# wvangansbeke/LaneDetection_End2End

Measured on AMD Instinct MI355X. Metric: images/sec fwd+bwd, 256x512 2-lane bs32, higher is better.
Workload: dtype f32; 1 GPU; BEV ERFNet + fused WLS fit + Area loss, 2 lanes, 256x512, batch 32 per GPU, fp32, train mode (BN batch stats, Dropout2d on), fwd+bwd, optimizer excluded; global_batch=32, parallelism=dp1, grad_allreduce=none

## Files before the change

### lanedetection_end2end_amd/_lib.py

```python
import ctypes
import os
from ctypes import c_char_p, c_double, c_int, c_long, c_size_t, c_void_p

import torch

_HERE = os.path.dirname(os.path.abspath(__file__))
LIB_PATH = os.path.join(_HERE, "liblanefit_hip.so")
_lib = None


class LaneFitLibraryError(RuntimeError):
    pass


def _declare(lib):
    P, I, L, D = c_void_p, c_int, c_long, c_double
    sig = {
        "lf_abi_version": (c_int, []),
        "lf_last_error": (c_char_p, []),
        "lf_wls_workspace_bytes": (c_size_t, [I, I, I]),
        "lf_wls_fwd": (I, [P, P, L, I, I, I, I, I, I, D, D, I, I, P, P, P, P, P, P]),
        "lf_wls_bwd": (I, [P, P, L, I, I, I, I, I, I, D, I, P, P, P, P, P]),
        "lf_gels_workspace_bytes": (c_size_t, [I, I]),
        "lf_gels_fwd": (I, [P, P, I, L, I, P, P, P, P, P]),
# ... 86 lines not shown
        "lf_wls_bwd_theta": (I, [P, P, L, P, P, I, I, I, I, I, I, D, I, P, P, P, P, P, P, P]),
        "lf_wls_bwd_grid": (I, [P, P, L, I, I, I, I, I, I, D, I, P, P, P, P, P]),
        "lf_lane_eval": (I, [P, P, P, P, P, P, L, P, I, I, I, I, I, D, D, P, P, P, P, P, P]),
        "lf_lane_decode_bev": (I, [P, I, P, P, P, P, L, P, P, I, D, P, P, I, I, I, I, I, I, I, I, I, I, P, P, P]),
        "lf_step_loss_workspace_bytes": (c_size_t, []),
        "lf_step_loss": (I, [I, I, I, I, I, I, I, P, L, I, P, P, L, I, P, P, P, P, P, P, P, I, D, D, P, P, P, P, P, P]),
        "lf_step_loss_bwd": (I, [P, I, L, L, P, P, P]),
        "lf_seg_step_workspace_bytes": (c_size_t, [I, I, I, I, I, I]),
        "lf_seg_step": (I, [P, P, P, P, L, P, I, I, I, I, I, I, I, D, D, I, P, P, P, P, P, P, P, P]),
        "lf_seg_step_bwd": (I, [P, L, P, P]),
        "lf_label_batch_bp": (I, [P, P, P, P, P, P, P, L, P, P, I, I, P, P, P, P, P, P, P, P, P]),
        "lf_label_batch_bev": (I, [P, P, P, P, P, L, P, P, I, P, P, P, P, P, P, P]),
    }
    dbg = {
        "lf_debug_set_split_any_size": (None, [I]),
        "lf_debug_set_bf16_lds": (None, [I]),
        "lf_debug_set_bf16_no_partial_fast": (None, [I]),
        "lf_debug_stride2_epi": (I, [I, I, P, P, P, P, I, P, P, P, P, I, I, I, I, I, P, P]),
        "lf_debug_set_ops_precision": (None, [I]),
        "lf_debug_conv1d_fwd_phases": (I, [P, P, P, P, I, I, I, I, I, I, P, P, P]),
        "lf_debug_conv1d_wgrad_phases": (I, [P, P, I, I, I, I, I, I, P, P, P]),
        "lf_debug_conv1d_fwd_pro": (I, [P, P, P, P, P, P, I, I, I, I, I, I, P, P]),
        "lf_debug_set_wgrad_ro": (None, [I, I, I]),
        "lf_debug_conv1d_bwd_data_epi3": (I, [P, P, P, P, P, P, P, I, I, I, I, I, I, P, P]),
        "lf_debug_conv1d_epi": (I, [P, P, P, P, I, I, P, P, P, P, P, P, I, I, I, I, I, I, P, P]),
        "lf_debug_conv1d_wgrad_pro": (I, [P, P, P, P, P, P, I, I, I, I, I, I, P, P]),
        "lf_debug_bias_residual_launches": (L, []),
        "lf_debug_partial_fast_launches": (L, []),
    }
    for table in (sig, dbg):
        for name, (res, args) in table.items():
            fn = getattr(lib, name)
            fn.restype = res
            fn.argtypes = args
    return sig


def exported_symbols():
    return list(_declare(load()).keys()) + list(_extra_symbols)


_extra_symbols = []


def load():
    global _lib
# ... 53 lines not shown
```

### lanedetection_end2end_amd/csrc/lf_conv.h

```cpp
#pragma once
#include "lf_common.h"

#define LF_MAX_TAPS 9
struct TapIdx { int v[LF_MAX_TAPS]; };

struct LfTapGeom {
    int N, Hl, Wl;
    int Hs, Ws, s_pix, s_choff;
    int ssh, ssw;
    int Hd, Wd, d_pix, d_choff;
    int dsh, dsw, dah, daw;
    int Cs, Cd;
    int ntaps;
    int tdh[LF_MAX_TAPS], tdw[LF_MAX_TAPS];
};

enum { LF_PRO_NONE = 0, LF_PRO_BNRELU = 1 };
enum {
    LF_EPI_RELU = 1,
    LF_EPI_MASK = 2,
    LF_EPI_ADD = 4,
    LF_EPI_STATS_SQ = 8,
    LF_EPI_MASKBN = 16,
    LF_EPI_STATS_XHAT = 32,
// ... 8 lines not shown
    int split;
    const void* wp48;
    const float* bias;
    float* dst;
    const float* pro_sc;
    const float* pro_sh;
    const float* mask_src;
    const float* add_src;
    const float* aux;
    const float* msc;
    const float* msh;
    const float* asc;
    const float* ash;
    const float* dm;
    float* stats;
    int stats_ld;
    unsigned long long* dbg;
};

void lf_tapgemm_set_split_any_size(int v);
void lf_tapgemm_set_bf16_lds(int v);
void lf_tapgemm_set_bf16_no_partial_fast(int v);
long lf_tapgemm_partial_fast_launches();
int lf_tapgemm_stat_rows(const LfTapGeom& g);
int lf_tapgemm_stat_rows_for(const LfTapGeom& g, const LfTapArgs& a);
int lf_tapgemm_launch(const LfTapGeom& g, const LfTapArgs& a, int pro, int epi, hipStream_t st);
int lf_tapgemm_launch_unordered(const LfTapGeom& g, const LfTapArgs& a, int pro, int epi, hipStream_t st);

struct LfWgradArgs {
    const float* x;
    const float* g;
    const float* pro_sc;
    const float* pro_sh;
    int s16;
    int split;
    float* partial;
    float* bias_partial;
    unsigned long long* dbg = nullptr;
};
int lf_tapwgrad_splits(const LfTapGeom& g);
int lf_tapwgrad_splits_bound(const LfTapGeom& g, int s16);
int lf_tapwgrad_splits_for(const LfTapGeom& g, const LfWgradArgs& a, int pro);
int lf_tapwgrad_launch(const LfTapGeom& g, const LfWgradArgs& a, int pro, hipStream_t st);

bool lf_tapwgrad_ro_ok(const LfTapGeom& g, int s16);
int lf_tapwgrad_ro_rows_bound(const LfTapGeom& g);
// ... 49 lines not shown
```

### lanedetection_end2end_amd/csrc/lf_conv.hip

```cpp
#include <stdlib.h>
#include <string.h>

#include <atomic>
#include <map>
#include <mutex>
#include <tuple>
#include <utility>

#include <hip/hip_ext.h>

#include "lf_conv.h"
#include "lf_ldsdma.h"
#include "lf_types.h"

typedef float f32x4 __attribute__((ext_vector_type(4)));

namespace {

constexpr int MT = 4;
constexpr int WG_WAVES = 4;
constexpr int PIX_PER_WG = WG_WAVES * MT * 16;

__device__ __forceinline__ f32x4 ldg4(const float* p) { return *reinterpret_cast<const f32x4*>(p); }
typedef unsigned u32x4v __attribute__((vector_size(16)));
// ... 51 lines not shown
}
template <int CTRL>
__device__ __forceinline__ float dpp_mov(float v) {
    return __builtin_bit_cast(float, __builtin_amdgcn_update_dpp(0, __builtin_bit_cast(int, v), CTRL, 0xf, 0xf, false));
}
__device__ __forceinline__ f32x4 bcast16(f32x4 v) {
    f32x4 r;
    r.x = dpp_mov<0x150>(v.x); r.y = dpp_mov<0x150>(v.y); r.z = dpp_mov<0x150>(v.z); r.w = dpp_mov<0x150>(v.w);
    return r;
}
__device__ __forceinline__ float sum16(float v) {
    v += dpp_mov<0xB1>(v);
    v += dpp_mov<0x4E>(v);
    v += dpp_mov<0x124>(v);
    v += dpp_mov<0x128>(v);
    return v;
}

#define LF_EPI_GROUPS 1
#define LF_EPI_ONE_TILE false
#define LF_EPI_TID threadIdx.x
#define LF_EPI_ROW1 false
#define LF_EPI_PIVOT true
#define LF_TAPGEMM_EPILOGUE \
      \
    const bool stats = (epi & (LF_EPI_STATS_SQ | LF_EPI_STATS_XHAT)) != 0; \
    constexpr bool NOBIAS = EPIC >= 0 && !(EPIC & LF_EPI_BIAS) && (EPIC & (LF_EPI_MASK | LF_EPI_ADD | LF_EPI_MASKBN | LF_EPI_STATS_XHAT)) != 0; \
    constexpr int NC = (NT % 2 == 0 && !LF_EPI_ONE_TILE) ? 2 : 1; \
     \
    constexpr bool HOISTM = HOISTV && !(EPIC >= 0 && (EPIC & LF_EPI_MASKBN) && (EPIC & LF_EPI_STATS_XHAT)); \
    __builtin_amdgcn_s_setprio(3);    \
    const __amdgpu_buffer_rsrc_t r_dst = make_rsrc(a.dst, 0xffffffffu), r_add = make_rsrc(a.add_src, 0xffffffffu), \
                                 r_msk = make_rsrc(a.mask_src, 0xffffffffu), r_aux = make_rsrc(a.aux, 0xffffffffu), \
                                 r_bias = make_rsrc(a.bias, 0xffffffffu), r_msc = make_rsrc(a.msc, 0xffffffffu), \
                                 r_msh = make_rsrc(a.msh, 0xffffffffu), r_dm = make_rsrc(a.dm, 0xffffffffu); \
     \
    f32x4 s1[NT], s2[NT], bs[NOBIAS ? 1 : NT], hv[HOISTV ? NT : 1][2], piv[LF_EPI_PIVOT ? NT : 1]; \
_Pragma("unroll") \
    for (int n = 0; n < NT; ++n) { \
        const int co = cob + n * 16 + kq * 4; \
        s1[n] = zero4(); s2[n] = zero4(); piv[LF_EPI_PIVOT ? n : 0] = zero4(); \
        if constexpr (!NOBIAS) bs[n] = a.bias ? ldb4(r_bias, co * 4u, 0u) : zero4(); \
        if (HOISTV) { \
            if (HOISTM && (epi & LF_EPI_MASKBN)) { hv[n][0] = ldb4(r_msc, co * 4u, 0u); hv[n][1] = ldb4(r_msh, co * 4u, 0u); } \
        } \
    } \
_Pragma("unroll") \
    for (int m = 0; m < MT; ++m) { \
        const unsigned dbase = (unsigned)(((pn[m] * g.Hd + pi[m] * g.dsh + g.dah) * g.Wd + pj[m] * g.dsw + g.daw) * g.d_pix + g.d_choff + cob + kq * 4); \
_Pragma("unroll") \
        for (int n0 = 0; n0 < NT; n0 += NC) { \
        f32x4 la[NC], lm[NC], lx[NC], ld[NC]; \
_Pragma("unroll") \
        for (int j = 0; j < NC; ++j) { \
            const int n = n0 + j; \
            if (epi & LF_EPI_ADD) la[j] = epi_ld<S16>(r_add, dbase + n * 16); \
            if (epi & LF_EPI_MASK) lm[j] = epi_ld<S16>(r_msk, dbase + n * 16); \
            if (epi & (LF_EPI_MASKBN | LF_EPI_STATS_XHAT)) lx[j] = epi_ld<S16>(r_aux, dbase + n * 16); \
            if ((epi & LF_EPI_STATS_XHAT) && a.dm && !LF_EPI_ROW1) ld[j] = ldb4(r_dm, (unsigned)(pn[m] * g.Cd + cob + n * 16 + kq * 4) * 4u, 0u); \
        } \
_Pragma("unroll") \
        for (int j = 0; j < NC; ++j) { \
            const int n = n0 + j; \
            f32x4 v = acc[n][m]; \
            if constexpr (!NOBIAS) v += bs[n]; \
            if (epi & LF_EPI_ADD) v += la[j]; \
            if (epi & LF_EPI_MASK) v = keep_pos(v, lm[j]); \
            const int co = cob + n * 16 + kq * 4;    \
            if (epi & LF_EPI_MASKBN) v = keep_pos(v, lx[j] * (HOISTM ? hv[HOISTV ? n : 0][0] : ldb4(r_msc, co * 4u, 0u)) + (HOISTM ? hv[HOISTV ? n : 0][1] : ldb4(r_msh, co * 4u, 0u))); \
            if (epi & LF_EPI_RELU) v = S16 ? relu_keep_nan(v) : max0(v); \
            if (S16) v = round_bf16(v);    \
            if (pv[m]) epi_st<S16>(r_dst, dbase + n * 16, v); \
            if (!pv[m]) v = zero4(); \
            if (epi & LF_EPI_STATS_SQ) { \
                if (LF_EPI_PIVOT && m == 0) piv[LF_EPI_PIVOT ? n : 0] = bcast16(v); \
                f32x4 dv = LF_EPI_PIVOT ? v - piv[LF_EPI_PIVOT ? n : 0] : v; \
                if (!pv[m]) dv = zero4(); \
                s1[n] += dv; s2[n] += dv * dv; \
            } \
            if (epi & LF_EPI_STATS_XHAT) { \
                const f32x4 gm = (a.dm && !LF_EPI_ROW1) ? v * ld[j] : v; \
                s1[n] += gm; s2[n] += gm * lx[j];       \
            } \
        } \
        } \
    } \
    if (LF_EPI_ROW1 && (epi & LF_EPI_STATS_XHAT) && a.dm) { \
         \
_Pragma("unroll") \
        for (int n = 0; n < NT; ++n) { \
            const f32x4 dmv = ldb4(r_dm, (unsigned)(pn[0] * g.Cd + cob + n * 16 + kq * 4) * 4u, 0u); \
            s1[n] *= dmv; s2[n] *= dmv; \
        } \
    } \
    if (stats) { \
         \
        const int EW = wave & 3, EG = wave >> 2; \
        __shared__ float sred[LF_EPI_GROUPS][WG_WAVES][NT][4][8]; \
_Pragma("unroll") \
        for (int n = 0; n < NT; ++n) { \
            f32x4 r1, r2; \
            r1.x = sum16(s1[n].x); r1.y = sum16(s1[n].y); r1.z = sum16(s1[n].z); r1.w = sum16(s1[n].w); \
            r2.x = sum16(s2[n].x); r2.y = sum16(s2[n].y); r2.z = sum16(s2[n].z); r2.w = sum16(s2[n].w); \
            if (epi & LF_EPI_STATS_SQ) {       \
                const unsigned lf_t0 = (bx * (unsigned)(WG_WAVES * LF_EPI_GROUPS) + (unsigned)wave) * 64u; \
                const float nw = lf_t0 < npix ? (float)min(npix - lf_t0, 64u) : 0.f; \
                const float rn = nw > 0.f ? 1.f / nw : 0.f; \
                r2 = r2 - r1 * r1 * rn; \
                r2.x = fmaxf(r2.x, 0.f); r2.y = fmaxf(r2.y, 0.f); r2.z = fmaxf(r2.z, 0.f); r2.w = fmaxf(r2.w, 0.f); \
                if (LF_EPI_PIVOT) r1 = r1 + piv[LF_EPI_PIVOT ? n : 0] * nw; \
            } \
            if (pl == 0) { \
                float* d = sred[EG][EW][n][kq]; \
                d[0] = r1.x; d[1] = r1.y; d[2] = r1.z; d[3] = r1.w; d[4] = r2.x; d[5] = r2.y; d[6] = r2.z; d[7] = r2.w; \
            } \
        } \
        __syncthreads(); \
        if ((LF_EPI_TID & 255) < NT * 4 * 8) { \
            const int tg = LF_EPI_TID >> 8, tt = LF_EPI_TID & 255; \
            const int j = tt & 7, q = (tt >> 3) & 3, n = tt >> 5; \
            float v = sred[tg][0][n][q][j] + sred[tg][1][n][q][j] + sred[tg][2][n][q][j] + sred[tg][3][n][q][j]; \
            if ((epi & LF_EPI_STATS_SQ) && j >= 4) {       \
                const unsigned lf_tb = (bx * (unsigned)LF_EPI_GROUPS + (unsigned)tg) * (unsigned)(WG_WAVES * 64); \
                float nwv[4], sw[4], nt = 0.f, st = 0.f; \
_Pragma("unroll") \
                for (int w = 0; w < 4; ++w) { \
                    const unsigned t0w = lf_tb + (unsigned)w * 64u; \
                    nwv[w] = t0w < npix ? (float)min(npix - t0w, 64u) : 0.f; \
                    sw[w] = sred[tg][w][n][q][j - 4]; \
                    nt += nwv[w]; st += sw[w]; \
                } \
                const float mg = nt > 0.f ? st / nt : 0.f; \
_Pragma("unroll") \
                for (int w = 0; w < 4; ++w) \
                    if (nwv[w] > 0.f) { const float dmw = sw[w] / nwv[w] - mg; v += nwv[w] * dmw * dmw; } \
            } \
            const int co = cob + n * 16 + q * 4 + (j & 3); \
            a.stats[((long)(j >> 2) * g.Cd + co) * a.stats_ld + ((long)bx * LF_EPI_GROUPS + tg)] = v;       \
        } \
    } \

extern __shared__ __attribute__((aligned(16))) unsigned char lf_tap_lds[];
constexpr size_t LF_TAP_LDS_PER_TAP = (size_t)WG_WAVES * 64 * (sizeof(uint4) + sizeof(unsigned));

template <int NT, int PROC, int EPIC = -1, bool ROW1 = false, bool DBG = false>
__global__ __launch_bounds__(256, (EPIC >= 0 || NT < 4) ? 2 : 1) void tapgemm_kernel(const LfTapGeom g, const LfTapArgs a, const int pro, const int epi_rt) {
    const int epi = EPIC >= 0 ? EPIC : epi_rt;
    constexpr bool S16 = false, HOISTV = EPIC >= 0;
    unsigned long long tstamp[4] = {0ull, 0ull, 0ull, 0ull};
    if constexpr (DBG) tstamp[0] = __builtin_amdgcn_s_memrealtime();
    const unsigned npix = (unsigned)(g.N * g.Hl * g.Wl);
    const int cob = blockIdx.y * NT * 16;
    const unsigned ntiles = (npix + PIX_PER_WG - 1) / PIX_PER_WG;
    unsigned t_first = blockIdx.x, t_stride = gridDim.x, t_end = ntiles;
    if ((gridDim.x & 7u) == 0 && (ntiles & 7u) == 0) {
        const unsigned per = ntiles >> 3;
        t_first = (blockIdx.x & 7u) * per + (blockIdx.x >> 3); t_stride = gridDim.x >> 3; t_end = (blockIdx.x & 7u) * per + per;
    }
    for (unsigned bx = t_first; bx < t_end; bx += t_stride) {
    unsigned tid = threadIdx.x;
    asm volatile("" : "+v"(tid));
    const int lane = tid & 63, wave = tid >> 6;
    const int pl = lane & 15, kq = lane >> 4;
// ... 171 lines not shown
    LF_TAPGEMM_EPILOGUE
#undef LF_EPI_ONE_TILE
#define LF_EPI_ONE_TILE false
#undef LF_EPI_TID
#define LF_EPI_TID threadIdx.x
#undef LF_EPI_ROW1
#define LF_EPI_ROW1 false
    if (stats && bx + t_stride < t_end) __syncthreads();
    __builtin_amdgcn_s_setprio(0);
    }
    if constexpr (DBG) {
        asm volatile("s_waitcnt vmcnt(0)" ::: "memory");
        tstamp[3] = __builtin_amdgcn_s_memrealtime();
        const int lane = threadIdx.x & 63, wave = threadIdx.x >> 6;
        if (lane == 0 && a.dbg) {
            unsigned long long* d = a.dbg + ((unsigned long long)(blockIdx.y * gridDim.x + blockIdx.x) * WG_WAVES + wave) * 8;
            d[0] = tstamp[0]; d[1] = tstamp[1]; d[2] = tstamp[2]; d[3] = tstamp[3];
            unsigned hwid, xcc;
            asm volatile("s_getreg_b32 %0, hwreg(HW_REG_HW_ID)" : "=s"(hwid));
            asm volatile("s_getreg_b32 %0, hwreg(HW_REG_XCC_ID)" : "=s"(xcc));
            d[4] = (unsigned long long)hwid | ((unsigned long long)xcc << 32);
        }
    }
}

typedef __bf16 bf16x8 __attribute__((ext_vector_type(8)));
typedef unsigned u32x4 __attribute__((ext_vector_type(4)));

__device__ __forceinline__ bf16x8 cvt_bf16x8(f32x4 lo, f32x4 hi) {
    bf16x8 r;
    r[0] = (__bf16)lo.x; r[1] = (__bf16)lo.y; r[2] = (__bf16)lo.z; r[3] = (__bf16)lo.w;
    r[4] = (__bf16)hi.x; r[5] = (__bf16)hi.y; r[6] = (__bf16)hi.z; r[7] = (__bf16)hi.w;
    return r;
}

template <int NT, int PROC, int EPIC = -1, bool FAST = false>
__global__ __launch_bounds__(256, 2) void tapgemm_bf16_kernel(const LfTapGeom g, const LfTapArgs a, const int pro, const int epi_rt) {
    static_assert(!FAST || PROC == 0, "FAST: the out-of-range zero must be the operand itself");
    const int epi = EPIC >= 0 ? EPIC : epi_rt;
    constexpr bool HOISTV = true, S16 = true;
    const int lane = threadIdx.x & 63, wave = threadIdx.x >> 6;
    const int pl = lane & 15, kq = lane >> 4;
    const unsigned npix = (unsigned)(g.N * g.Hl * g.Wl);
    const int cob = blockIdx.y * NT * 16;
    unsigned bx = blockIdx.x;
    if ((gridDim.x & 7u) == 0) bx = (bx & 7u) * (gridDim.x >> 3) + (bx >> 3);
// ... 1356 lines not shown
bool lf_tapgemm_split_ok(const LfTapGeom& g) {
    const long npix = (long)g.N * g.Hl * g.Wl;
    const long wgs = npix / (2 * PIX_PER_WG) * (g.Cd / 64);
    return g.Cs % 32 == 0 && g.Cd % 64 == 0 && g.s_pix % 4 == 0 && g.s_choff % 4 == 0 && npix % (2 * PIX_PER_WG) == 0 &&
           (wgs >= 192 || g_split_any_size);
}

int lf_tapgemm_stat_rows(const LfTapGeom& g) {
    const long npix = (long)g.N * g.Hl * g.Wl;
    return lf_cdiv(npix, PIX_PER_WG);
}
int lf_tapgemm_stat_rows_for(const LfTapGeom& g, const LfTapArgs& a) {
    (void)a;
    return lf_cdiv((long)g.N * g.Hl * g.Wl, PIX_PER_WG);
}

namespace {
std::mutex g_launch_state_mutex;
int current_device() {
    int dev = 0;
    return hipGetDevice(&dev) == hipSuccess ? dev : -1;
}
template <typename K>
int resident_workgroups(K kernel, size_t lds) {
    static std::map<std::tuple<int, const void*, size_t>, int> cache;
    const int dev = current_device();
    const std::tuple<int, const void*, size_t> key(dev, reinterpret_cast<const void*>(kernel), lds);
    std::lock_guard<std::mutex> lock(g_launch_state_mutex);
    auto it = cache.find(key);
    if (it != cache.end()) return it->second;
    int cus = 0, nb = 0;
    if (dev < 0 || hipDeviceGetAttribute(&cus, hipDeviceAttributeMultiprocessorCount, dev) != hipSuccess ||
        hipOccupancyMaxActiveBlocksPerMultiprocessor(&nb, kernel, 256, lds) != hipSuccess || nb < 1 || cus < 1)
        return cache[key] = 1 << 30;
    return cache[key] = nb * cus;
}
bool allow_big_lds(const void* kernel, int bytes) {
    static std::map<std::pair<int, const void*>, bool> done;
    const std::pair<int, const void*> key(current_device(), kernel);
    std::lock_guard<std::mutex> lock(g_launch_state_mutex);
    auto it = done.find(key);
    if (it != done.end()) return it->second;
    return done[key] = hipFuncSetAttribute(kernel, hipFuncAttributeMaxDynamicSharedMemorySize, bytes) == hipSuccess;
}
thread_local unsigned g_launch_flags = 0;
template <typename K>
void launch_tapgemm(K kernel, dim3 grid, size_t lds, hipStream_t st, const LfTapGeom& g, const LfTapArgs& a, int pro, int epi) {
    const unsigned res = (unsigned)resident_workgroups(kernel, lds) / grid.y;
    if (grid.x > res && res >= 8) grid.x = res & ~7u;
    if (g_launch_flags) hipExtLaunchKernelGGL(kernel, grid, dim3(256), (unsigned)lds, st, nullptr, nullptr, g_launch_flags, g, a, pro, epi);
    else hipLaunchKernelGGL(kernel, grid, dim3(256), lds, st, g, a, pro, epi);
}
template <int EPIV, bool DBGV = false>
void launch_bf16_ring(unsigned nitems, hipStream_t st, const LfTapGeom& g, const LfTapArgs& a, int pro, int epi) {
    auto kern = tapgemm_bf16_ring_kernel<EPIV, DBGV>;
    const size_t ring_lds = (size_t)LB_STAGES * LB_STAGE_BYTES;
// ... 4 lines not shown
}
template <int CBV, int EPIV, int PROV = 0>
bool launch_bf16_wl(unsigned nitems, hipStream_t st, const LfTapGeom& g, const LfTapArgs& a, int pro, int epi) {
    auto kern = tapgemm_bf16_wl_kernel<CBV, EPIV, PROV>;
    const size_t lds = WlCfg<CBV, EPIV, PROV>::LDS;
    if (!allow_big_lds(reinterpret_cast<const void*>(kern), 160 * 1024 - 4096)) return false;
    unsigned gx = nitems;
    const unsigned res = (unsigned)resident_workgroups(kern, lds);
    if (gx > res && res >= 8) gx = res & ~7u;
    hipLaunchKernelGGL(kern, dim3(gx), dim3(256), lds, st, g, a, pro, epi);
    return true;
}
template <int EPIV>
bool launch_bf16_wv(unsigned ntiles, hipStream_t st, const LfTapGeom& g, const LfTapArgs& a, int pro, int epi) {
    auto kern = tapgemm_bf16_wv_kernel<EPIV>;
    const size_t lds = WvCfg<EPIV>::LDS;
    if (!allow_big_lds(reinterpret_cast<const void*>(kern), 160 * 1024 - 4096)) return false;
    unsigned gx = ntiles;
    const unsigned res = (unsigned)resident_workgroups(kern, lds);
    if (gx > res && res >= 8) gx = res & ~7u;
    hipLaunchKernelGGL(kern, dim3(gx), dim3(256), lds, st, g, a, pro, epi);
    return true;
}
}

int lf_tapgemm_launch_unordered(const LfTapGeom& g, const LfTapArgs& a, int pro, int epi, hipStream_t st) {
    g_launch_flags = hipExtAnyOrderLaunch;
    const int rc = lf_tapgemm_launch(g, a, pro, epi, st);
    g_launch_flags = 0;
    return rc;
}

int lf_tapgemm_launch(const LfTapGeom& g, const LfTapArgs& a, int pro, int epi, hipStream_t st) {
    LF_REQUIRE(g.Cs % 16 == 0 && g.Cd % 16 == 0, "tapgemm: channels must be multiples of 16 (Cs=%d Cd=%d)", g.Cs, g.Cd);
    LF_REQUIRE(g.s_pix % 4 == 0 && g.s_choff % 4 == 0 && g.d_pix % 4 == 0 && g.d_choff % 4 == 0, "tapgemm: unaligned channel layout");
    LF_REQUIRE(g.ntaps >= 1 && g.ntaps <= LF_MAX_TAPS, "tapgemm: bad tap count %d", g.ntaps);
    const long npix = (long)g.N * g.Hl * g.Wl;
    LF_REQUIRE(npix < (1L << 30), "tapgemm: too many pixels (%ld)", npix);
    const int nt = pick_nt(g.Cd);
    dim3 grid(lf_cdiv(npix, PIX_PER_WG), g.Cd / (16 * nt));
    LF_REQUIRE((long)g.N * g.Hs * g.Ws * g.s_pix * 4 < (long)LF_OOB, "tapgemm: source tensor too large for 32-bit byte offsets");
    LF_REQUIRE((long)g.N * g.Hd * g.Wd * g.d_pix * 4 < (long)LF_OOB, "tapgemm: destination tensor too large for 32-bit byte offsets");
#define LF_TG(NTV)                                                                                                       \
    do {                                                                                                                 \
        if (pro == LF_PRO_BNRELU) launch_tapgemm(tapgemm_kernel<NTV, 1>, grid, tap_lds, st, g, a, pro, epi);  \
        else launch_tapgemm(tapgemm_kernel<NTV, 0>, grid, tap_lds, st, g, a, pro, epi);                       \
    } while (0)
// ... 178 lines not shown
            else if (epis == LF_EPI_STATS_SQ) hipLaunchKernelGGL((tapgemm_bf16_kernel<1, 0, LF_EPI_STATS_SQ, true>), grid, dim3(256), 0, st, g, a, pro, epi);
            else if (epis == LF_EPI_RELU) hipLaunchKernelGGL((tapgemm_bf16_kernel<1, 0, LF_EPI_RELU, true>), grid, dim3(256), 0, st, g, a, pro, epi);
            else hipLaunchKernelGGL((tapgemm_bf16_kernel<1, 0, LF_EPI_ADD, true>), grid, dim3(256), 0, st, g, a, pro, epi);
            if (g.Cs % 32 != 0) ++g_part_fast_launches;
        } else
        switch (nt) {
            case 4: LF_TG16(4); break;
            case 3: LF_TG16(3); break;
            case 2: LF_TG16(2); break;
            default: LF_TG16(1); break;
        }
#undef LF_TG16
#undef LF_TG16F
        LF_CHECK_LAUNCH("tapgemm_bf16");
        return 0;
    }
    if (a.dbg) {
        LF_REQUIRE(nt == 4 && pro == LF_PRO_NONE && epi == 0 && !a.wp16, "tapgemm: phase stamps are compiled into the plain fp32 convolution only");
        if ((g.Wl & 63) == 0) hipLaunchKernelGGL((tapgemm_kernel<4, 0, 0, true, true>), grid, dim3(256), tap_lds, st, g, a, pro, epi);
        else hipLaunchKernelGGL((tapgemm_kernel<4, 0, 0, false, true>), grid, dim3(256), tap_lds, st, g, a, pro, epi);
        LF_CHECK_LAUNCH("tapgemm (stamps)");
        return 0;
    }
    switch (nt) {
        case 4:
            if (pro == LF_PRO_BNRELU && epi == LF_EPI_RELU) LF_TG4(1, LF_EPI_RELU);
            else if (pro == LF_PRO_BNRELU) LF_TG4(1, -1);
            else switch (epis) {
                case 0: LF_TG4(0, 0); break;
                case LF_EPI_RELU: LF_TG4(0, LF_EPI_RELU); break;
                case LF_EPI_MASK: LF_TG4(0, LF_EPI_MASK); break;
                case LF_EPI_ADD: LF_TG4(0, LF_EPI_ADD); break;
                case LF_EPI_STATS_SQ: LF_TG4(0, LF_EPI_STATS_SQ); break;
                case LF_EPI_MASK | LF_EPI_STATS_XHAT: LF_TG4(0, LF_EPI_MASK | LF_EPI_STATS_XHAT); break;
                case LF_EPI_ADD | LF_EPI_MASK | LF_EPI_STATS_XHAT: LF_TG4(0, LF_EPI_ADD | LF_EPI_MASK | LF_EPI_STATS_XHAT); break;
                case LF_EPI_MASKBN | LF_EPI_STATS_XHAT: LF_TG4(0, LF_EPI_MASKBN | LF_EPI_STATS_XHAT); break;
                case BRES: LF_TG4(0, BRES); ++g_bres_launches; break;
                default: LF_TG4(0, -1); break;
            }
            break;
        case 3: LF_TG(3); break;
        case 2: LF_TG(2); break;
        default:
            {
#define LF_LEAN(PROV, EPIV) hipLaunchKernelGGL((tapgemm_lean_kernel<1, PROV, EPIV>), grid, dim3(256), 0, st, g, a, pro, epi)
                if (pro == LF_PRO_BNRELU && epi == LF_EPI_RELU) LF_LEAN(1, LF_EPI_RELU);
// ... 1125 lines not shown
```

### lanedetection_end2end_amd/csrc/lf_debug.h

```cpp
#pragma once
#ifdef __cplusplus
extern "C" {
#endif
void lf_debug_set_split_any_size(int v);
void lf_debug_set_bf16_lds(int v);
void lf_debug_set_bf16_no_partial_fast(int v);
long lf_debug_partial_fast_launches(void);
void lf_debug_set_ops_precision(int mode);
int lf_debug_conv1d_fwd_phases(const float* x, const float* w, const float* bias, float* y, int N, int H, int W, int C,
                               int axis, int dilation, float* scratch, unsigned long long* dbg, void* stream);
int lf_debug_conv1d_fwd_pro(const float* x, const float* w, const float* bias, const float* sc, const float* sh, float* y, int N, int H,
                            int W, int C, int axis, int dilation, float* scratch, void* stream);
void lf_debug_set_wgrad_ro(int mode, int cap64, int cap128);
int lf_debug_conv1d_wgrad_pro(const float* x, const float* gy, const float* sc, const float* sh, float* gw, float* gb, int N, int H, int W,
                              int C, int axis, int dilation, float* scratch, void* stream);
int lf_debug_conv1d_bwd_data_epi3(const float* gy, const float* w, const float* mask_src, const float* add_src, const float* aux,
                                  float* gx, float* stats, int N, int H, int W, int C, int axis, int dilation, float* scratch, void* stream);
int lf_debug_conv1d_epi(const float* src, const float* w, const float* bias, float* dst, int transposed, int epi, const float* mask_src,
                        const float* add_src, const float* aux, const float* msc, const float* msh, float* stats, int N, int H, int W, int C,
                        int axis, int dilation, float* scratch, void* stream);
int lf_debug_stride2_epi(int kind, int phase, const float* src, const float* w, const float* bias, float* dst, int epi, const float* mask_src,
                         const float* add_src, const float* aux, float* stats, int N, int H, int W, int Cin, int Cout, float* scratch,
                         void* stream);
long lf_debug_bias_residual_launches(void);
int lf_debug_conv1d_wgrad_phases(const float* x, const float* gy, int N, int H, int W, int C, int axis, int dilation,
                                 float* scratch, unsigned long long* dbg, void* stream);
#ifdef __cplusplus
}
#endif
```

### lanedetection_end2end_amd/csrc/lf_ops.hip

```cpp
#include "lf_conv.h"
#include "lf_debug.h"
#include "lf_plan.h"

namespace {

TapIdx conv1d_taps(int flip) {
    TapIdx ti;
    memset(&ti, 0, sizeof(ti));
    for (int t = 0; t < 3; ++t) ti.v[t] = flip ? 2 - t : t;
    return ti;
}

__global__ __launch_bounds__(256) void pack_one_kernel(const float* __restrict__ w, float* __restrict__ dst, int Kc, int Nc,
                                                      int ntaps, long sk, long sn, const TapIdx ti) {
    const long total = (long)ntaps * Kc * Nc;
    for (long i = (long)blockIdx.x * 256 + threadIdx.x; i < total; i += (long)gridDim.x * 256) {
        const int k4 = (int)(i & 3);
        long r = i >> 2;
        const int n = (int)(r % Nc);
        r /= Nc;
        const int kb = (int)(r % (Kc >> 2));
        const int t = (int)(r / (Kc >> 2));
        dst[i] = w[(kb * 4 + k4) * sk + n * sn + ti.v[t]];
    }
// ... 55 lines not shown
    }
    a.wp = scratch;
}

LfTapGeom conv1d_geom(int N, int H, int W, int C, int axis, int d) {
    LfTapGeom g;
    memset(&g, 0, sizeof(g));
    g.N = N; g.Hl = H; g.Wl = W; g.Hs = H; g.Ws = W; g.s_pix = C; g.ssh = 1; g.ssw = 1;
    g.Hd = H; g.Wd = W; g.d_pix = C; g.dsh = 1; g.dsw = 1; g.Cs = C; g.Cd = C; g.ntaps = 3;
    for (int t = 0; t < 3; ++t) { g.tdh[t] = axis == 0 ? (t - 1) * d : 0; g.tdw[t] = axis == 1 ? (t - 1) * d : 0; }
    return g;
}

}

extern "C" {

void lf_debug_set_split_any_size(int v) { lf_tapgemm_set_split_any_size(v); }
void lf_debug_set_bf16_lds(int v) { lf_tapgemm_set_bf16_lds(v); }
void lf_debug_set_bf16_no_partial_fast(int v) { lf_tapgemm_set_bf16_no_partial_fast(v); }
void lf_debug_set_ops_precision(int mode) { g_ops_bf16 = (mode == 2 || mode == 9) ? mode : 0; }

void lf_debug_set_wgrad_ro(int mode, int cap64, int cap128) { lf_tapwgrad_ro_set(mode, cap64, cap128); }
long lf_debug_bias_residual_launches(void) { return lf_tapgemm_bias_residual_launches(); }
long lf_debug_partial_fast_launches(void) { return lf_tapgemm_partial_fast_launches(); }

int lf_debug_conv1d_fwd_phases(const float* x, const float* w, const float* bias, float* y, int N, int H, int W, int C,
                               int axis, int dilation, float* scratch, unsigned long long* dbg, void* stream) {
    hipStream_t st = (hipStream_t)stream;
    const LfTapGeom g = conv1d_geom(N, H, W, C, axis, dilation);
    LfTapArgs a;
    memset(&a, 0, sizeof(a));
    pack_conv1d(a, w, scratch, C, 3L, 3L * C, 0, st);
    a.src = x; a.bias = bias; a.dst = y; a.dbg = dbg;
    return lf_tapgemm_launch(g, a, LF_PRO_NONE, 0, st);
}

int lf_debug_conv1d_fwd_pro(const float* x, const float* w, const float* bias, const float* sc, const float* sh, float* y, int N, int H,
                            int W, int C, int axis, int dilation, float* scratch, void* stream) {
    LF_REQUIRE(x && w && y && sc && sh && scratch, "lf_debug_conv1d_fwd_pro: null pointer");
    hipStream_t st = (hipStream_t)stream;
    const LfTapGeom g = conv1d_geom(N, H, W, C, axis, dilation);
    LfTapArgs a;
    memset(&a, 0, sizeof(a));
    pack_conv1d(a, w, scratch, C, 3L, 3L * C, 0, st);
    a.src = x; a.bias = bias; a.dst = y; a.pro_sc = sc; a.pro_sh = sh;
// ... 141 lines not shown
```

### profiles/summarize_traffic_step.py

```python
import json
import os
import re
import sqlite3
import sys

FAMILIES = (("conv forward + data gradient (tap-GEMM kernels)", r"^tapgemm"), ("weight gradient (+ its reductions)", r"^tapwgrad|^wgrad_reduce|^rows_reduce|stem_wgrad|head_wgrad"),
            ("BatchNorm / element-wise passes", r"bn_|pool_|stem_fwd|head_fwd|head_bwd|pack_weights"), ("fit + losses", r"wls_|area_loss|backproj|ce_|mse_|seg_maps|trapezoid"))


def short(name):
    name = re.sub(r"\(anonymous namespace\)::", "", name)
    name = re.sub(r"^void ", "", name)
    m = re.match(r"_ZN12_GLOBAL__N_1\d+([A-Za-z_0-9]+?)I", name)
    return m.group(1) if m else re.sub(r"[<(].*$", "", name)


def per_kernel(db, counter):
    cur = sqlite3.connect(db).cursor()
    agg = {}
    for name, cn, value in cur.execute("select kernel_name, counter_name, value from counters_collection"):
        if cn != counter:
            continue
        a = agg.setdefault(short(name), [0, 0.0])
        a[0] += 1
        a[1] += value
    return agg


def main(fetch_db, write_db, key, commit, digest):
# ... 32 lines not shown
```

Measured before the change: 1994 images/sec.

## Add persistent streaming fp32 tap-GEMM kernel for 3-tap square convs

```diff
diff --git a/lanedetection_end2end_amd/_lib.py b/lanedetection_end2end_amd/_lib.py
--- a/lanedetection_end2end_amd/_lib.py
+++ b/lanedetection_end2end_amd/_lib.py
@@ -132,6 +132,7 @@
         "lf_debug_conv1d_wgrad_phases": (I, [P, P, I, I, I, I, I, I, P, P, P]),
         "lf_debug_conv1d_fwd_pro": (I, [P, P, P, P, P, P, I, I, I, I, I, I, P, P]),
         "lf_debug_set_wgrad_ro": (None, [I, I, I]),
+        "lf_debug_set_fp32_stream": (None, [I, I]),
         "lf_debug_conv1d_bwd_data_epi3": (I, [P, P, P, P, P, P, P, I, I, I, I, I, I, P, P]),
         "lf_debug_conv1d_epi": (I, [P, P, P, P, I, I, P, P, P, P, P, P, I, I, I, I, I, I, P, P]),
         "lf_debug_conv1d_wgrad_pro": (I, [P, P, P, P, P, P, I, I, I, I, I, I, P, P]),
diff --git a/lanedetection_end2end_amd/csrc/lf_conv.h b/lanedetection_end2end_amd/csrc/lf_conv.h
--- a/lanedetection_end2end_amd/csrc/lf_conv.h
+++ b/lanedetection_end2end_amd/csrc/lf_conv.h
@@ -54,6 +54,7 @@
 void lf_tapgemm_set_bf16_lds(int v);
 void lf_tapgemm_set_bf16_no_partial_fast(int v);
 long lf_tapgemm_partial_fast_launches();
+void lf_tapgemm_set_fp32_stream(int mode, int max_workgroups);
 int lf_tapgemm_stat_rows(const LfTapGeom& g);
 int lf_tapgemm_stat_rows_for(const LfTapGeom& g, const LfTapArgs& a);
 int lf_tapgemm_launch(const LfTapGeom& g, const LfTapArgs& a, int pro, int epi, hipStream_t st);
diff --git a/lanedetection_end2end_amd/csrc/lf_conv.hip b/lanedetection_end2end_amd/csrc/lf_conv.hip
--- a/lanedetection_end2end_amd/csrc/lf_conv.hip
+++ b/lanedetection_end2end_amd/csrc/lf_conv.hip
@@ -97,14 +97,16 @@
 #define LF_EPI_TID threadIdx.x
 #define LF_EPI_ROW1 false
 #define LF_EPI_PIVOT true
-#define LF_TAPGEMM_EPILOGUE \
+#define LF_EPI_ACC(n, m) acc[n][m]
+#define LF_EPI_FIRST(m) ((m) == 0)
+#define LF_EPI_ROW_OK(tg) true
+#define LF_EPI_HEAD \
       \
     const bool stats = (epi & (LF_EPI_STATS_SQ | LF_EPI_STATS_XHAT)) != 0; \
     constexpr bool NOBIAS = EPIC >= 0 && !(EPIC & LF_EPI_BIAS) && (EPIC & (LF_EPI_MASK | LF_EPI_ADD | LF_EPI_MASKBN | LF_EPI_STATS_XHAT)) != 0; \
     constexpr int NC = (NT % 2 == 0 && !LF_EPI_ONE_TILE) ? 2 : 1; \
      \
     constexpr bool HOISTM = HOISTV && !(EPIC >= 0 && (EPIC & LF_EPI_MASKBN) && (EPIC & LF_EPI_STATS_XHAT)); \
-    __builtin_amdgcn_s_setprio(3);    \
     const __amdgpu_buffer_rsrc_t r_dst = make_rsrc(a.dst, 0xffffffffu), r_add = make_rsrc(a.add_src, 0xffffffffu), \
                                  r_msk = make_rsrc(a.mask_src, 0xffffffffu), r_aux = make_rsrc(a.aux, 0xffffffffu), \
                                  r_bias = make_rsrc(a.bias, 0xffffffffu), r_msc = make_rsrc(a.msc, 0xffffffffu), \
@@ -119,9 +121,9 @@
         if (HOISTV) { \
             if (HOISTM && (epi & LF_EPI_MASKBN)) { hv[n][0] = ldb4(r_msc, co * 4u, 0u); hv[n][1] = ldb4(r_msh, co * 4u, 0u); } \
         } \
-    } \
-_Pragma("unroll") \
-    for (int m = 0; m < MT; ++m) { \
+    }
+#define LF_EPI_TILE(m) \
+    { \
         const unsigned dbase = (unsigned)(((pn[m] * g.Hd + pi[m] * g.dsh + g.dah) * g.Wd + pj[m] * g.dsw + g.daw) * g.d_pix + g.d_choff + cob + kq * 4); \
 _Pragma("unroll") \
         for (int n0 = 0; n0 < NT; n0 += NC) { \
@@ -137,7 +139,7 @@
 _Pragma("unroll") \
         for (int j = 0; j < NC; ++j) { \
             const int n = n0 + j; \
-            f32x4 v = acc[n][m]; \
+            f32x4 v = LF_EPI_ACC(n, m); \
             if constexpr (!NOBIAS) v += bs[n]; \
             if (epi & LF_EPI_ADD) v += la[j]; \
             if (epi & LF_EPI_MASK) v = keep_pos(v, lm[j]); \
@@ -148,7 +150,7 @@
             if (pv[m]) epi_st<S16>(r_dst, dbase + n * 16, v); \
             if (!pv[m]) v = zero4(); \
             if (epi & LF_EPI_STATS_SQ) { \
-                if (LF_EPI_PIVOT && m == 0) piv[LF_EPI_PIVOT ? n : 0] = bcast16(v); \
+                if (LF_EPI_PIVOT && LF_EPI_FIRST(m)) piv[LF_EPI_PIVOT ? n : 0] = bcast16(v); \
                 f32x4 dv = LF_EPI_PIVOT ? v - piv[LF_EPI_PIVOT ? n : 0] : v; \
                 if (!pv[m]) dv = zero4(); \
                 s1[n] += dv; s2[n] += dv * dv; \
@@ -159,7 +161,8 @@
             } \
         } \
         } \
-    } \
+    }
+#define LF_EPI_TAIL \
     if (LF_EPI_ROW1 && (epi & LF_EPI_STATS_XHAT) && a.dm) { \
          \
 _Pragma("unroll") \
@@ -191,7 +194,7 @@
             } \
         } \
         __syncthreads(); \
-        if ((LF_EPI_TID & 255) < NT * 4 * 8) { \
+        if ((LF_EPI_TID & 255) < NT * 4 * 8 && LF_EPI_ROW_OK(LF_EPI_TID >> 8)) { \
             const int tg = LF_EPI_TID >> 8, tt = LF_EPI_TID & 255; \
             const int j = tt & 7, q = (tt >> 3) & 3, n = tt >> 5; \
             float v = sred[tg][0][n][q][j] + sred[tg][1][n][q][j] + sred[tg][2][n][q][j] + sred[tg][3][n][q][j]; \
@@ -213,7 +216,13 @@
             const int co = cob + n * 16 + q * 4 + (j & 3); \
             a.stats[((long)(j >> 2) * g.Cd + co) * a.stats_ld + ((long)bx * LF_EPI_GROUPS + tg)] = v;       \
         } \
-    } \
+    }
+#define LF_TAPGEMM_EPILOGUE \
+    __builtin_amdgcn_s_setprio(3);    \
+    LF_EPI_HEAD \
+_Pragma("unroll") \
+    for (int m = 0; m < MT; ++m) LF_EPI_TILE(m) \
+    LF_EPI_TAIL
 
 extern __shared__ __attribute__((aligned(16))) unsigned char lf_tap_lds[];
 constexpr size_t LF_TAP_LDS_PER_TAP = (size_t)WG_WAVES * 64 * (sizeof(uint4) + sizeof(unsigned));
@@ -431,6 +440,151 @@
             d[4] = (unsigned long long)hwid | ((unsigned long long)xcc << 32);
         }
     }
+}
+
+template <int CS, int PROC, int EPIC, int G>
+__global__ __launch_bounds__(256 * G, G == 1 ? 2 : 1) void tapstream_kernel(const LfTapGeom g, const LfTapArgs a) {
+    constexpr int NT = 4, NCG = CS / 16, NS = 3 * NCG, R = 8;
+    constexpr int epi = EPIC;
+    constexpr bool S16 = false, HOISTV = true;
+    static_assert((4 * NS) % R == 0 && R <= NS && NS % 2 == 0, "ring positions and K-step pairs must be compile-time");
+    const unsigned npix = (unsigned)(g.N * g.Hl * g.Wl);
+    const int cob = blockIdx.y * 64;
+    const unsigned ntiles = (npix + PIX_PER_WG - 1) / PIX_PER_WG, nunits = (ntiles + G - 1) / G;
+    unsigned u_first = blockIdx.x, u_stride = gridDim.x, u_end = nunits;
+    if ((gridDim.x & 7u) == 0 && (nunits & 7u) == 0) {
+        const unsigned per = nunits >> 3;
+        u_first = (blockIdx.x & 7u) * per + (blockIdx.x >> 3); u_stride = gridDim.x >> 3; u_end = (blockIdx.x & 7u) * per + per;
+    }
+    const int lane = threadIdx.x & 63, wave = threadIdx.x >> 6;
+    const int pl = lane & 15, kq = lane >> 4;
+    const unsigned wtile = (unsigned)__builtin_amdgcn_readfirstlane(wave);
+
+
+    f32x4* const wl = reinterpret_cast<f32x4*>(lf_tap_lds);
+    float* const pvec = reinterpret_cast<float*>(wl + NS * 256);
+    struct WT { int n0, i0, j0; bool v; };
+    auto coords = [&](unsigned u, bool live) -> WT {
+        const unsigned tile0 = (u * (unsigned)(4 * G) + wtile) * 64u;
+        WT c;
+        c.v = live && tile0 < npix;
+        const unsigned q = c.v ? tile0 : 0u;
+        const unsigned r = q / (unsigned)g.Wl;
+        c.j0 = __builtin_amdgcn_readfirstlane((int)(q - r * (unsigned)g.Wl));
+        c.n0 = __builtin_amdgcn_readfirstlane((int)(r / (unsigned)g.Hl));
+        c.i0 = __builtin_amdgcn_readfirstlane((int)r) - c.n0 * g.Hl;
+        return c;
+    };
+    auto xoff = [&](const WT& c, int sub, int t, bool& in) -> unsigned {
+        const int sy = c.i0 * g.ssh + g.tdh[t], sx = (c.j0 + sub * 16 + pl) * g.ssw + g.tdw[t];
+        in = c.v && sy >= 0 && sy < g.Hs && sx >= 0 && sx < g.Ws;
+        const int syc = min(max(sy, 0), g.Hs - 1), sxc = min(max(sx, 0), g.Ws - 1);
+        const unsigned o = (unsigned)(((c.n0 * g.Hs + syc) * g.Ws + sxc) * g.s_pix + g.s_choff + kq * 4) * 4u;
+        return (PROC == 0 && !in) ? LF_OOB : o;
+    };
+    const __amdgpu_buffer_rsrc_t rx = make_rsrc(a.src, (unsigned)min((long)g.N * g.Hs * g.Ws * g.s_pix * 4, (long)LF_OOB));
+    auto xload = [&](const WT& c, int p) -> f32x4 {
+        const int k = p % NS;
+        bool in;
+        const unsigned o = xoff(c, p / NS, k / NCG, in);
+        return ldb4(rx, o, (unsigned)(k % NCG) * 64u);
+    };
+
+    f32x4 ring[R], wn[NT];
+    WT cur = coords(u_first, u_first < u_end);
+#pragma unroll
+    for (int p = 0; p < R; ++p) ring[p] = xload(cur, p);
+    {
+        const __amdgpu_buffer_rsrc_t rw = make_rsrc(a.wp, (unsigned)(3 * CS * CS * 4));
+        for (int idx = threadIdx.x; idx < NS * 256; idx += 256 * G) {
+            const int col = idx & 63, row = idx >> 6;
+            wl[((row >> 2) * 4 + (col >> 4)) * 64 + (row & 3) * 16 + (col & 15)] = ldb4(rw, (unsigned)(row * CS + cob + col) * 16u, 0u);
+        }
+        if constexpr (PROC == LF_PRO_BNRELU) {
+            const __amdgpu_buffer_rsrc_t rsc = make_rsrc(a.pro_sc, CS * 4u), rsh = make_rsrc(a.pro_sh, CS * 4u);
+            for (int i = threadIdx.x; i < 2 * CS; i += 256 * G)
+                pvec[i] = __uint_as_float(__builtin_amdgcn_raw_buffer_load_b32(i < CS ? rsc : rsh, (i < CS ? i : i - CS) * 4, 0, 0));
+        }
+    }
+    __syncthreads();
+#pragma unroll
+    for (int n = 0; n < NT; ++n) wn[n] = wl[n * 64 + lane];
+
+#undef LF_EPI_GROUPS
+#define LF_EPI_GROUPS G
+#undef LF_EPI_ROW1
+#define LF_EPI_ROW1 true
+#undef LF_EPI_ACC
+#define LF_EPI_ACC(n, m) acc[n]
+#undef LF_EPI_FIRST
+#define LF_EPI_FIRST(m) (sub == 0)
+#undef LF_EPI_ROW_OK
+#define LF_EPI_ROW_OK(tg) (bx * (unsigned)G + (unsigned)(tg) < ntiles)
+    LF_EPI_HEAD
+    for (unsigned bx = u_first; bx < u_end; bx += u_stride) {
+        const WT nxt = coords(bx + u_stride, bx + u_stride < u_end);
+        const int pn[1] = {cur.n0}, pi[1] = {cur.i0};
+        const bool pv[1] = {cur.v};
+#pragma unroll
+        for (int sub = 0; sub < 4; ++sub) {
+            f32x4 acc[NT], accl[NT];
+#pragma unroll
+            for (int k = 0; k < NS; ++k) {
+                const int p = sub * NS + k, cg = k % NCG;
+                f32x4 w[NT];
+#pragma unroll
+                for (int n = 0; n < NT; ++n) w[n] = wn[n];
+#pragma unroll
+                for (int n = 0; n < NT; ++n) wn[n] = wl[(((k + 1) % NS) * 4 + n) * 64 + lane];
+                f32x4 x = ring[p % R];
+                if constexpr (PROC == LF_PRO_BNRELU) {
+                    bool in;
+                    (void)xoff(cur, sub, k / NCG, in);
+                    const f32x4 sc = *reinterpret_cast<const f32x4*>(pvec + cg * 16 + kq * 4);
+                    const f32x4 sh = *reinterpret_cast<const f32x4*>(pvec + CS + cg * 16 + kq * 4);
+                    f32x4 v = max0(x * sc + sh);
+                    v.x = in ? v.x : 0.f; v.y = in ? v.y : 0.f; v.z = in ? v.z : 0.f; v.w = in ? v.w : 0.f;
+                    x = v;
+                }
+                if (k % 2 == 0) {
+#pragma unroll
+                    for (int n = 0; n < NT; ++n) {
+                        if (k == 0) accl[n] = zero4();
+                        else { accl[n] += acc[n]; asm volatile("" : "+v"(accl[n])); }
+                        acc[n] = __builtin_amdgcn_mfma_f32_16x16x4f32(w[n][0], x[0], zero4(), 0, 0, 0);
+                    }
+                }
+#pragma unroll
+                for (int s = (k % 2 == 0) ? 1 : 0; s < 4; ++s)
+#pragma unroll
+                    for (int n = 0; n < NT; ++n) acc[n] = __builtin_amdgcn_mfma_f32_16x16x4f32(w[n][s], x[s], acc[n], 0, 0, 0);
+                if (p + R < 4 * NS) ring[p % R] = xload(cur, p + R);
+                else ring[p % R] = xload(nxt, p + R - 4 * NS);
+                __builtin_amdgcn_sched_barrier(0);
+            }
+#pragma unroll
+            for (int n = 0; n < NT; ++n) acc[n] += accl[n];
+            const int pj[1] = {cur.j0 + sub * 16 + pl};
+            LF_EPI_TILE(0)
+        }
+        LF_EPI_TAIL
+        if (stats) {
+#pragma unroll
+            for (int n = 0; n < NT; ++n) { s1[n] = zero4(); s2[n] = zero4(); }
+            if (bx + u_stride < u_end) __syncthreads();
+        }
+        cur = nxt;
+    }
+#undef LF_EPI_GROUPS
+#define LF_EPI_GROUPS 1
+#undef LF_EPI_ROW1
+#define LF_EPI_ROW1 false
+#undef LF_EPI_ACC
+#define LF_EPI_ACC(n, m) acc[n][m]
+#undef LF_EPI_FIRST
+#define LF_EPI_FIRST(m) ((m) == 0)
+#undef LF_EPI_ROW_OK
+#define LF_EPI_ROW_OK(tg) true
 }
 
 typedef __bf16 bf16x8 __attribute__((ext_vector_type(8)));
@@ -1833,7 +1987,7 @@
     return hipGetDevice(&dev) == hipSuccess ? dev : -1;
 }
 template <typename K>
-int resident_workgroups(K kernel, size_t lds) {
+int resident_workgroups(K kernel, size_t lds, int block = 256) {
     static std::map<std::tuple<int, const void*, size_t>, int> cache;
     const int dev = current_device();
     const std::tuple<int, const void*, size_t> key(dev, reinterpret_cast<const void*>(kernel), lds);
@@ -1842,7 +1996,7 @@
     if (it != cache.end()) return it->second;
     int cus = 0, nb = 0;
     if (dev < 0 || hipDeviceGetAttribute(&cus, hipDeviceAttributeMultiprocessorCount, dev) != hipSuccess ||
-        hipOccupancyMaxActiveBlocksPerMultiprocessor(&nb, kernel, 256, lds) != hipSuccess || nb < 1 || cus < 1)
+        hipOccupancyMaxActiveBlocksPerMultiprocessor(&nb, kernel, block, lds) != hipSuccess || nb < 1 || cus < 1)
         return cache[key] = 1 << 30;
     return cache[key] = nb * cus;
 }
@@ -1893,7 +2047,41 @@
     hipLaunchKernelGGL(kern, dim3(gx), dim3(256), lds, st, g, a, pro, epi);
     return true;
 }
-}
+std::atomic<int> g_stream_mode{1}, g_stream_cap{0};
+enum { LF_STREAM_RELU = 1, LF_STREAM_STATS = 2, LF_STREAM_MASK = 4, LF_STREAM_PRO = 8, LF_STREAM_X48 = 16, LF_STREAM_X38 = 32 };
+constexpr int g_stream_routed[2] = {LF_STREAM_RELU | LF_STREAM_STATS | LF_STREAM_MASK | LF_STREAM_PRO | LF_STREAM_X48 | LF_STREAM_X38,
+                                    0};
+template <int CS, int PROV, int EPIV>
+bool launch_tapstream(hipStream_t st, const LfTapGeom& g, const LfTapArgs& a) {
+    constexpr int G = CS == 128 ? 2 : 1;
+    auto kern = tapstream_kernel<CS, PROV, EPIV, G>;
+    const size_t lds = (size_t)3 * (CS / 16) * 4096 + (PROV == LF_PRO_BNRELU ? 2 * CS * sizeof(float) : 0);
+    if (!allow_big_lds(reinterpret_cast<const void*>(kern), 160 * 1024 - 4096)) return false;
+    const unsigned ntiles = (unsigned)lf_cdiv((long)g.N * g.Hl * g.Wl, PIX_PER_WG);
+    dim3 grid((ntiles + G - 1) / G, CS / 64);
+    const unsigned res = (unsigned)resident_workgroups(kern, lds, 256 * G) / grid.y;
+    if (grid.x > res && res >= 8) grid.x = res & ~7u;
+    const unsigned cap = (unsigned)g_stream_cap.load();
+    if (cap > 0 && grid.x > cap) grid.x = cap;
+    if (g_launch_flags) hipExtLaunchKernelGGL(kern, grid, dim3(256 * G), (unsigned)lds, st, nullptr, nullptr, g_launch_flags, g, a);
+    else hipLaunchKernelGGL(kern, grid, dim3(256 * G), lds, st, g, a);
+    return true;
+}
+template <int CS>
+bool route_tapstream(int variant, hipStream_t st, const LfTapGeom& g, const LfTapArgs& a) {
+    switch (variant) {
+        case LF_STREAM_RELU: return launch_tapstream<CS, 0, LF_EPI_RELU>(st, g, a);
+        case LF_STREAM_STATS: return launch_tapstream<CS, 0, LF_EPI_STATS_SQ>(st, g, a);
+        case LF_STREAM_MASK: return launch_tapstream<CS, 0, LF_EPI_MASK>(st, g, a);
+        case LF_STREAM_PRO: return launch_tapstream<CS, 1, LF_EPI_RELU>(st, g, a);
+        case LF_STREAM_X48: if constexpr (CS == 64) return launch_tapstream<CS, 0, LF_EPI_MASKBN | LF_EPI_STATS_XHAT>(st, g, a); else return false;
+        case LF_STREAM_X38: if constexpr (CS == 64) return launch_tapstream<CS, 0, LF_EPI_ADD | LF_EPI_MASK | LF_EPI_STATS_XHAT>(st, g, a); else return false;
+        default: return false;
+    }
+}
+}
+
+void lf_tapgemm_set_fp32_stream(int mode, int max_workgroups) { g_stream_mode = mode; g_stream_cap = max_workgroups > 0 ? max_workgroups : 0; }
 
 int lf_tapgemm_launch_unordered(const LfTapGeom& g, const LfTapArgs& a, int pro, int epi, hipStream_t st) {
     g_launch_flags = hipExtAnyOrderLaunch;
@@ -2118,6 +2306,16 @@
         LF_CHECK_LAUNCH("tapgemm (stamps)");
         return 0;
     }
+    if (g_stream_mode.load() != 0 && nt == 4 && g.ntaps == 3 && g.Cs == g.Cd && (g.Cs == 64 || g.Cs == 128) && (g.Wl & 63) == 0) {
+        const int variant = pro == LF_PRO_BNRELU ? (epi == LF_EPI_RELU ? LF_STREAM_PRO : 0)
+                          : epis == LF_EPI_RELU ? LF_STREAM_RELU : epis == LF_EPI_STATS_SQ ? LF_STREAM_STATS : epis == LF_EPI_MASK ? LF_STREAM_MASK
+                          : epis == (LF_EPI_MASKBN | LF_EPI_STATS_XHAT) ? LF_STREAM_X48 : epis == (LF_EPI_ADD | LF_EPI_MASK | LF_EPI_STATS_XHAT) ? LF_STREAM_X38 : 0;
+        if (variant && (g_stream_mode.load() == 2 || (g_stream_routed[g.Cs == 128] & variant)) &&
+            (g.Cs == 64 ? route_tapstream<64>(variant, st, g, a) : route_tapstream<128>(variant, st, g, a))) {
+            LF_CHECK_LAUNCH("tapstream");
+            return 0;
+        }
+    }
     switch (nt) {
         case 4:
             if (pro == LF_PRO_BNRELU && epi == LF_EPI_RELU) LF_TG4(1, LF_EPI_RELU);
diff --git a/lanedetection_end2end_amd/csrc/lf_debug.h b/lanedetection_end2end_amd/csrc/lf_debug.h
--- a/lanedetection_end2end_amd/csrc/lf_debug.h
+++ b/lanedetection_end2end_amd/csrc/lf_debug.h
@@ -12,6 +12,7 @@
 int lf_debug_conv1d_fwd_pro(const float* x, const float* w, const float* bias, const float* sc, const float* sh, float* y, int N, int H,
                             int W, int C, int axis, int dilation, float* scratch, void* stream);
 void lf_debug_set_wgrad_ro(int mode, int cap64, int cap128);
+void lf_debug_set_fp32_stream(int mode, int max_workgroups);
 int lf_debug_conv1d_wgrad_pro(const float* x, const float* gy, const float* sc, const float* sh, float* gw, float* gb, int N, int H, int W,
                               int C, int axis, int dilation, float* scratch, void* stream);
 int lf_debug_conv1d_bwd_data_epi3(const float* gy, const float* w, const float* mask_src, const float* add_src, const float* aux,
diff --git a/lanedetection_end2end_amd/csrc/lf_ops.hip b/lanedetection_end2end_amd/csrc/lf_ops.hip
--- a/lanedetection_end2end_amd/csrc/lf_ops.hip
+++ b/lanedetection_end2end_amd/csrc/lf_ops.hip
@@ -101,6 +101,7 @@
 void lf_debug_set_ops_precision(int mode) { g_ops_bf16 = (mode == 2 || mode == 9) ? mode : 0; }
 
 void lf_debug_set_wgrad_ro(int mode, int cap64, int cap128) { lf_tapwgrad_ro_set(mode, cap64, cap128); }
+void lf_debug_set_fp32_stream(int mode, int max_workgroups) { lf_tapgemm_set_fp32_stream(mode, max_workgroups); }
 long lf_debug_bias_residual_launches(void) { return lf_tapgemm_bias_residual_launches(); }
 long lf_debug_partial_fast_launches(void) { return lf_tapgemm_partial_fast_launches(); }
 
diff --git a/profiles/summarize_per_launch.py b/profiles/summarize_per_launch.py
--- /dev/null
+++ b/profiles/summarize_per_launch.py
@@ -0,0 +1,34 @@
+import re
+import sqlite3
+import sys
+
+
+def short(name):
+    name = re.sub(r"\(anonymous namespace\)::", "", name)
+    return re.sub(r"^void ", "", re.sub(r"\(.*$", "", name))[:70]
+
+
+def main(path, pat=r"^tap(gemm|stream)_kernel"):
+    cur = sqlite3.connect(path).cursor()
+    cols = [r[1] for r in cur.execute("pragma table_info(kernels)")]
+    name_col = "name" if "name" in cols else [c for c in cols if "name" in c][0]
+    dims = [c for c in cols if re.search(r"^(grid|workgroup)(_size)?_?[xy]$", c, re.I)]
+    if not dims:
+        print("# no grid columns among %s" % cols)
+    agg = {}
+    for row in cur.execute("select %s, start, end%s from kernels" % (name_col, "".join(", " + c for c in dims))):
+        k = short(row[0])
+        if not re.search(pat, k):
+            continue
+        a = agg.setdefault((k,) + tuple(row[3:]), [])
+        a.append(row[2] - row[1])
+    print("# %s" % path)
+    print("%-72s %-22s %6s %9s %9s %9s %9s" % ("kernel", "/".join(dims), "calls", "avg_us", "median_us", "min_us", "max_us"))
+    for key, v in sorted(agg.items(), key=lambda kv: -sum(kv[1])):
+        v.sort()
+        print("%-72s %-22s %6d %9.2f %9.2f %9.2f %9.2f" % (key[0], "/".join(str(d) for d in key[1:]), len(v), sum(v) / len(v) / 1e3,
+                                                         v[len(v) // 2] / 1e3, v[0] / 1e3, v[-1] / 1e3))
+
+
+if __name__ == "__main__":
+    main(*sys.argv[1:3])
diff --git a/profiles/summarize_traffic_step.py b/profiles/summarize_traffic_step.py
--- a/profiles/summarize_traffic_step.py
+++ b/profiles/summarize_traffic_step.py
@@ -4,7 +4,7 @@
 import sqlite3
 import sys
 
-FAMILIES = (("conv forward + data gradient (tap-GEMM kernels)", r"^tapgemm"), ("weight gradient (+ its reductions)", r"^tapwgrad|^wgrad_reduce|^rows_reduce|stem_wgrad|head_wgrad"),
+FAMILIES = (("conv forward + data gradient (tap-GEMM kernels)", r"^tapgemm|^tapstream"), ("weight gradient (+ its reductions)", r"^tapwgrad|^wgrad_reduce|^rows_reduce|stem_wgrad|head_wgrad"),
             ("BatchNorm / element-wise passes", r"bn_|pool_|stem_fwd|head_fwd|head_bwd|pack_weights"), ("fit + losses", r"wls_|area_loss|backproj|ce_|mse_|seg_maps|trapezoid"))
 
 
```

After: 2018 images/sec (median of 6 runs). 1.2% higher.
